# zynthbox/libzl

Measured on AMD Instinct MI355X. Metric: voice-samples/sec at 1024 voices x 256-frame blocks; % HBM roofline, higher is better.
Workload: dtype f32

## Files before the change

libzl_amd/build.py:

```python
from __future__ import annotations

import os
import shutil
import subprocess
import sys

ROOT = os.path.dirname(os.path.dirname(os.path.abspath(__file__)))
CSRC = os.path.join(ROOT, "libzl_amd", "csrc")
LIBDIR = os.path.join(ROOT, "libzl_amd", "lib")
LIB = os.path.join(LIBDIR, "libzlhip.so")

HIP_SOURCES = ["zl_kernels.hip", "zl_stretch.hip", "zl_overview.hip", "zl_decode.hip", "zl_engine.cpp", "zl_libzl.cpp", "zl_group.cpp"]
HEADERS = ["zl_types.h", "zl_arena.h", "zl_plan.h", "zl_order.h", "zl_pair.h", "zl_launch.h", "zl_render.h", "zl_kernels.h", "zl_host.h", "zl_sched.h", "zl_handoff.h", "zl_stretch.h", "zl_overview.h", "zl_decode.h", "zl_group.h", "zl_member.h",
           os.path.join("..", "..", "include", "zlhip.h"), os.path.join("..", "..", "include", "libzl_hotpath.h")]


def _hipcc() -> str:
    for cand in (os.environ.get("HIPCC"), shutil.which("hipcc"), "/opt/rocm/bin/hipcc"):
        if cand and os.path.exists(cand):
            return cand
    raise RuntimeError("hipcc not found (needed to build libzlhip.so for gfx950)")


def _stale(target: str, deps: list[str]) -> bool:
    if not os.path.exists(target):
        return True
    t = os.path.getmtime(target)
    return any(os.path.exists(d) and os.path.getmtime(d) > t for d in deps)


def build_variant(name: str, flags: list, verbose: bool = False) -> str:
    global LIB
    saved, LIB = LIB, os.path.join(LIBDIR, f"libzlhip_{name}.so")
    try:
        return _build_engine(False, verbose, list(flags))
    finally:
        LIB = saved


def build_engine(force: bool = False, verbose: bool = False, stamps: bool = False) -> str:
    global LIB
    if stamps:
        out = os.path.join(LIBDIR, "libzlhip_stamps.so")
        saved, LIB = LIB, out
        try:
            return _build_engine(force, verbose, ["-DZL_STAMPS"])
        finally:
            LIB = saved
    return _build_engine(force, verbose, [])


_INC = os.path.join("..", "..", "include")
SOURCE_DEPS = {
    "zl_kernels.hip": ["zl_types.h", "zl_plan.h", "zl_render.h", "zl_order.h", "zl_pair.h", "zl_launch.h", "zl_kernels.h"],
    "zl_stretch.hip": ["zl_types.h", "zl_stretch.h"],
    "zl_overview.hip": ["zl_types.h", "zl_overview.h"],
    "zl_decode.hip": ["zl_types.h", "zl_decode.h"],
    "zl_engine.cpp": ["zl_types.h", "zl_arena.h", "zl_plan.h", "zl_render.h", "zl_order.h", "zl_pair.h", "zl_launch.h", "zl_host.h", "zl_kernels.h", "zl_member.h", "zl_stretch.h", "zl_overview.h", "zl_decode.h", os.path.join(_INC, "zlhip.h")],
    "zl_group.cpp": ["zl_types.h", "zl_plan.h", "zl_order.h", "zl_pair.h", "zl_launch.h", "zl_host.h", "zl_kernels.h", "zl_member.h", "zl_group.h", os.path.join(_INC, "zlhip.h")],
    "zl_libzl.cpp": ["zl_render.h", "zl_types.h", "zl_sched.h", "zl_handoff.h", "zl_stretch.h", os.path.join(_INC, "zlhip.h"), os.path.join(_INC, "libzl_hotpath.h")],
}


def _write_kernel_resources(remarks: str, path: str) -> None:
    import re
    rows, cur = [], None
    for line in remarks.splitlines():
        m = re.search(r"remark:\s+Function Name: (\S+)", line)
        if m:
            cur = {"name": m.group(1)}
            rows.append(cur)
            continue
        m = re.search(r"remark:\s+(VGPRs|ScratchSize \[bytes/lane\]|Occupancy \[waves/SIMD\]|LDS Size \[bytes/block\]|VGPRs Spill): (\d+)", line)
        if m and cur is not None:
            cur[m.group(1).split(" ")[0] + ("Spill" if "Spill" in m.group(1) else "")] = int(m.group(2))
    with open(path, "w") as f:
        for r in rows:
            f.write(f"{r['name']} vgprs={r.get('VGPRs', -1)} scratch={r.get('ScratchSize', -1)} waves={r.get('Occupancy', -1)} lds={r.get('LDS', -1)} vgpr_spill={r.get('VGPRsSpill', -1)}\n")


def _build_engine(force: bool, verbose: bool, extra: list) -> str:
    names = [s for s in HIP_SOURCES if os.path.exists(os.path.join(CSRC, s))]
# ... 142 lines not shown


def build_pair_harness(force: bool = False) -> str:
    return _build_harness("zl_pair_host", "pair_host.cpp", ["zl_pair.h"], ["-Wall"], force)


def build_group_harness(force: bool = False) -> str:
    return _build_harness("zl_group_host", "group_host.cpp", ["zl_types.h", "zl_plan.h", "zl_host.h", "zl_group.h", _ZLHIP_H], _NO_CONTRACT + ["-Wall", "-Wno-unused-function"], force)


def build_overview_harness(force: bool = False) -> str:
    return _build_harness("zl_overview_host", "overview_host.cpp", ["zl_types.h", "zl_overview.h"], ["-Wall"], force)


def build_decode_harness(force: bool = False) -> str:
    return _build_harness("zl_decode_host", "decode_host.cpp", ["zl_types.h", "zl_decode.h"], _NO_CONTRACT + ["-Wall"], force)


def build_arena_harness(force: bool = False) -> str:
    return _build_harness("zl_arena_host", "arena_host.cpp", ["zl_types.h", "zl_stretch.h", "zl_arena.h"], ["-Wall"], force)


def build_launch_harness(force: bool = False) -> str:
    return _build_harness("zl_launch_host", "launch_host.cpp", ["zl_types.h", "zl_order.h", "zl_pair.h", "zl_launch.h"], ["-Wall", "-Wno-unused-function"], force)


if __name__ == "__main__":
    force = "--force" in sys.argv
    print(build_engine(force=force, verbose=True))
    print(build_oracle(force=force))
```

libzl_amd/csrc/zl_engine.cpp:

```cpp
#include <hip/hip_runtime.h>
#include <sys/resource.h>

#include <algorithm>
#include <atomic>
#include <cmath>
#include <cstdio>
#include <cstdlib>
#include <chrono>
#include <cstring>
#include <mutex>
#include <string>
#include <utility>
#include <vector>

#include "../../include/zlhip.h"
#include "zl_arena.h"
#include "zl_host.h"
#include "zl_kernels.h"
#include "zl_member.h"
#include "zl_order.h"
#include "zl_pair.h"
#include "zl_plan.h"
#include "zl_overview.h"
#include "zl_decode.h"
// ... 1347 lines not shown
        ZL_HIP(e, hipMemsetAsync(e->dTrace, 0xff, need * sizeof(int32_t), s));
        A.trace = 1; traceBase = e->dTrace; e->traceK = nblocks; e->traceN = nframes;
#ifdef ZL_STAMPS
        A.trace = 0;
#endif
    }

    static const int windowMulEnv = [] { const char *v = std::getenv("ZL_WINDOW_MUL"); const int m = v ? std::atoi(v) : 0; return m < 0 ? 0 : (m > 64 ? 64 : m); }();
    bool cheap = nframes >= 256;
    for (const ZlHostVoice &hv : e->hc.voices) if (hv.isPlaying && !hv.cheapPlan) { cheap = false; break; }
    int windowMul = windowMulEnv;
    if (windowMul == 0) windowMul = cheap ? 4 : 1;
    const size_t mul = e->maxGroups > 1 ? 1 : (size_t)windowMul;
    std::vector<std::pair<int, int>> &wins = e->wins;
    zlhip_engine::CallSlot &prev = e->slots[(e->callIndex + 1u) & 1u];
    const bool behindPrev = prev.inflight && hipEventQuery(prev.done) == hipErrorNotReady;
    const char *fw = std::getenv("ZL_FIRST_WINDOW_FRAMES");
    const int fwFrames = fw ? std::atoi(fw) : 0;
    zl_plan_windows(nblocks, nframes, e->windowBlocks, e->windowFrames, e->windowCap, mul, e->ps[1].hdr != nullptr, behindPrev, fw ? &fwFrames : nullptr, wins);
    const int nwin = (int)wins.size();
    const int phaseMode = [] { const char *v = std::getenv("ZL_K2_PHASE_ORDER"); return v ? std::atoi(v) : 1; }();
    const double loopFrames = phaseMode == 1 ? e->hc.phase_order_loop_frames() : INFINITY;
    const int pairMode = [] { const char *v = std::getenv("ZL_K2_PAIR"); return v ? std::atoi(v) : 1; }();
    const int stageNorun = [] { const char *v = std::getenv("ZL_K2_STAGE_NORUN"); return v ? (std::atoi(v) != 0 ? 1 : 0) : 1; }();
    const bool direct = e->bnc.sink.on && e->bnc.sink.hostDev && A.groups == 1;
    const ZlK2Switches &k2sw = zl_k2_switches();
    auto k2Launch = [&](int K, bool orderTable) {
        ZlK2In in;
        in.mode = A.mode; in.N = nframes; in.K = K; in.B = A.B; in.groups = A.groups; in.NB = A.NB;
        in.staged = A.staged; in.trace = A.trace; in.ongrid = A.ongrid; in.fan = fan_out_dev != nullptr; in.host_out = direct;
        in.order_mode = phaseMode; in.call_blocks = nblocks; in.bounce = e->bnc.sink.on; in.order_table = orderTable; in.loop_frames = loopFrames;
        in.pair_mode = pairMode; in.cheap = cheap;
        return zl_k2_launch(in, k2sw);
    };
    {
        size_t need = 0;
        for (const auto &wk : wins) { const ZlK2Launch L = k2Launch(wk.second, true); if (L.order) need = std::max(need, zl_order_ints((int)L.gz, wk.second, e->V)); }
        if (need > e->ps[0].orderInts || (e->ps[1].hdr != nullptr && need > e->ps[1].orderInts)) {
            ZlQuiesce quiet(e);
            for (auto &q : e->ps) {
                if (need <= q.orderInts || q.hdr == nullptr) continue;
                if (q.order) ZL_HIP(e, hipFree(q.order));
                q.order = nullptr; q.orderInts = 0;
                ZL_HIP(e, dalloc(&q.order, need));
                q.orderInts = need;
            }
        }
    }
    const bool overlap = e->ps[1].hdr != nullptr && (nwin > 1 || behindPrev || e->bnc.active);
    hipStream_t ps = overlap ? e->planStream : s;
    if (e->lastPlanStream && e->lastPlanStream != ps && e->lastPlanEvent) ZL_HIP(e, hipStreamWaitEvent(ps, e->lastPlanEvent, 0));
    if (nblocks == 1) { A.inline_clock = 1; A.clock0 = c.hClocks[0]; A.fuse_assemble = 1; }
    if (fan_out_dev) {
        for (int b = 0; b < A.B; ++b) c.hPass[b] = pass_params(fan_params[b]);
        ZL_HIP(e, hipMemcpyAsync(c.dPass, c.hPass, (size_t)A.B * sizeof(ZlPassParams), hipMemcpyHostToDevice, ps));
// ... 28 lines not shown
        if (w > 0) { Aw.n_op_ranges = 0; Aw.ops = nullptr; Aw.op_ranges = nullptr; Aw.n_clip_edits = 0; Aw.clip_edits = nullptr; }
        if (ps != s && q.used) ZL_HIP(e, hipStreamWaitEvent(ps, q.renderedEv, 0));
        ZL_KERNEL(e, zl_launch_apply_ops(Aw, ps));
        ZL_KERNEL(e, zl_launch_plan(Aw, e->forceSlow, ps));
        if (ps != s && e->asmStream && !Aw.fuse_assemble) {
            ZL_HIP(e, hipEventRecord(q.k1done, ps));
            ZL_HIP(e, hipStreamWaitEvent(e->asmStream, q.k1done, 0));
            ZL_KERNEL(e, zl_launch_assemble(Aw, e->asmStream));
            if (L.order) ZL_KERNEL(e, zl_launch_order(Aw, q.order, (int)L.gz, stageNorun, e->asmStream));
            ZL_HIP(e, hipEventRecord(q.planned, e->asmStream));
            ZL_HIP(e, hipStreamWaitEvent(s, q.planned, 0));
        } else {
            if (!Aw.fuse_assemble) ZL_KERNEL(e, zl_launch_assemble(Aw, ps));
            if (L.order) ZL_KERNEL(e, zl_launch_order(Aw, q.order, (int)L.gz, stageNorun, ps));
            if (ps != s) {
                ZL_HIP(e, hipEventRecord(q.planned, ps));
                ZL_HIP(e, hipStreamWaitEvent(s, q.planned, 0));
            }
        }
        const bool k3 = !L.scans_levels;
        if (direct) { Aw.host_out = e->bnc.sink.hostDev; Aw.host_fmt = e->bnc.sink.pcm ? 1 : 0; Aw.host_total = (long long)e->bnc.sink.totalFrames; Aw.host_k0 = 0; }
        const bool closes = fusedReports && w == nwin - 1;
        if (fusedReports) { Aw.fused_reports = 1; Aw.rep_gain = e->dGain; Aw.rep_host = c.hReportsDev; Aw.rep_host_gain = c.hGainDev; Aw.rep_host_stats = c.hStatsDev; }
        Aw.pair = (L.kernel == ZL_K2_PAIR_RENDER || L.kernel == ZL_K2_PAIR_PHASE_RENDER) ? 1 : 0;
        hipEvent_t k2stop = closes ? c.done : (e->profiling ? c.evK2[2 * (size_t)w + 1] : nullptr);
        ZL_KERNEL(e, zl_launch_render(Aw, L, s, e->profiling ? c.evK2[2 * (size_t)w] : nullptr, k2stop));
        if (k3) ZL_KERNEL(e, zl_launch_finalize(Aw, nullptr, s));
        if (e->bnc.sink.on && !direct) { int d_ = bounce_deliver_window(e, A.bus, 0, Aw.B, Aw.k0, Aw.K, nblocks, nframes, s); if (d_ != ZLHIP_OK) return d_; }
        if (e->ps[1].hdr != nullptr) {
            if (k2stop && !k3) q.renderedEv = k2stop;
            else { ZL_HIP(e, hipEventRecord(q.rendered, s)); q.renderedEv = q.rendered; }
            q.used = true;
        }
    }
    c.windows = nwin;
    if (ps != s) { ZL_HIP(e, hipEventRecord(e->evPlanTail, ps)); e->lastPlanEvent = e->evPlanTail; }
    else e->lastPlanEvent = c.done;
    e->lastPlanStream = ps;
    if (e->ps[1].hdr != nullptr) e->setPhase = (phase + (unsigned)nwin) & 1u;
    if (fusedReports) {
        if (e->profiling) c.profiled = true;
    } else {
        ZL_KERNEL(e, zl_launch_reports(c.dReports, e->V, e->dGain, c.hReportsDev, c.hGainDev, c.dStats, c.hStatsDev, s, e->profiling ? nullptr : c.done));
        if (e->profiling) { ZL_HIP(e, hipEventRecord(c.evEnd, s)); c.profiled = true; ZL_HIP(e, hipEventRecord(c.done, s)); }
    }
    c.inflight = true;
    if (s != e->stream) e->joins[0] = c.done;
// ... 666 lines not shown
```

libzl_amd/csrc/zl_kernels.hip:

```cpp
#include <hip/hip_runtime.h>
#include <hip/hip_ext.h>
#include <algorithm>
#include <cstddef>
#include "zl_types.h"
#include "zl_plan.h"
#include "zl_render.h"
#include "zl_order.h"
#include "zl_pair.h"
#include "zl_kernels.h"

static __device__ __forceinline__ void zl_apply_clip_edit(const ZlBatch &A, const ZlClipEdit *ed, int lane)
{
    static_assert(offsetof(ZlClip, slice_pos) == ZL_CLIP_HEAD_BYTES && sizeof(ZlClip) % 16 == 0 && offsetof(ZlClipEdit, c) % 16 == 0, "clip record layout");
    const int clip = ed->clip;
    const int n16 = ed->full ? (int)(sizeof(ZlClip) / 16) : ZL_CLIP_HEAD_BYTES / 16;
    const uint4 *src = reinterpret_cast<const uint4 *>(&ed->c);
    uint4 *dst = reinterpret_cast<uint4 *>(const_cast<ZlClip *>(A.clips) + clip);
    for (int w = lane; w < n16; w += 64) dst[w] = src[w];
}

__global__ void zl_k0_apply_ops(const ZlBatch A)
{
    const int opGroups = (A.n_op_ranges + 63) / 64;
    if ((int)blockIdx.x >= opGroups) {
        zl_apply_clip_edit(A, A.clip_edits + ((int)blockIdx.x - opGroups), (int)threadIdx.x);
        return;
    }
    const int i = blockIdx.x * blockDim.x + threadIdx.x;
    if (i >= A.n_op_ranges) return;
    const ZlOpRange rg = A.op_ranges[i];
    ZlVoiceState st = A.voices[rg.voice];
// ... 107 lines not shown
    ZlOrderKey key;
    if (s_key == INT_MAX || !zl_order_setup(A.runs[s_key], K, A.N, key)) {
        for (int k = tid; k < K; k += 256) out[k] = k;
        return;
    }
    for (int b = tid; b < key.nbkt; b += 256) s_hist[b] = 0;
    __syncthreads();
    for (int k = tid; k < K; k += 256) atomicAdd(&s_hist[zl_order_bucket(key, k)], 1);
    __syncthreads();
    const int per = (key.nbkt + 255) / 256, b0 = tid * per, b1 = b0 + per < key.nbkt ? b0 + per : key.nbkt;
    int sum = 0;
    for (int b = b0; b < b1; ++b) sum += s_hist[b];
    s_part[tid] = sum;
    __syncthreads();
    for (int off = 1; off < 256; off <<= 1) {
        const int t = tid >= off ? s_part[tid - off] : 0;
        __syncthreads();
        s_part[tid] += t;
        __syncthreads();
    }
    int run = s_part[tid] - sum;
    for (int b = b0; b < b1; ++b) { const int c = s_hist[b]; s_hist[b] = run; run += c; }
    __syncthreads();
    for (int k = tid; k < K; k += 256) out[atomicAdd(&s_hist[zl_order_bucket(key, k)], 1)] = k;
}

static __device__ __forceinline__ int zl_sample_to_peak_int(float x)
{
    const float v = 131072.0f * x;
    int r;
    asm("v_cvt_i32_f32_e64 %0, |%1|" : "=v"(r) : "v"(v));
    return r;
}

template <int CTRL, int ROWMASK>
static __device__ __forceinline__ int zl_dpp_i(int ident, int v) { return __builtin_amdgcn_update_dpp(ident, v, CTRL, ROWMASK, 0xf, false); }
static __device__ __forceinline__ int zl_wave_max_nonneg(int v)
{
    int t;
    t = zl_dpp_i<0xB1, 0xf>(0, v);  v = t > v ? t : v;
    t = zl_dpp_i<0x4E, 0xf>(0, v);  v = t > v ? t : v;
    t = zl_dpp_i<0x114, 0xf>(0, v); v = t > v ? t : v;
    t = zl_dpp_i<0x118, 0xf>(0, v); v = t > v ? t : v;
    t = zl_dpp_i<0x142, 0xa>(0, v); v = t > v ? t : v;
    t = zl_dpp_i<0x143, 0xc>(0, v); v = t > v ? t : v;
    return __builtin_amdgcn_readlane(v, 63);
}
// ... 1372 lines not shown

    if (A.fused_reports && A.k0 + k == A.Ktot - 1) {
        __syncthreads();
        for (int v = v0 + (int)threadIdx.x; v < v1; v += (int)blockDim.x) {
            const uint4 *src = reinterpret_cast<const uint4 *>(&A.reports[v]);
            uint4 a = src[0];
            const uint4 b = src[1];
            a.z = __hip_atomic_load(&A.reports[v].peak_bits, __ATOMIC_RELAXED, __HIP_MEMORY_SCOPE_AGENT);
            const float gn = __uint_as_float(a.z) * 0.5f;
            A.rep_gain[v] = gn;
            if (A.rep_host) { uint4 *dst = reinterpret_cast<uint4 *>(&A.rep_host[v]); dst[0] = a; dst[1] = b; A.rep_host_gain[v] = gn; }
        }
        if (bus == 0 && threadIdx.x == 0 && A.rep_host_stats) {
            const unsigned long long sb = A.stats->source_bytes, sl = A.stats->slow_blocks, af = A.stats->active_frames;
            A.rep_host_stats->source_bytes = sb; A.rep_host_stats->slow_blocks = sl; A.rep_host_stats->active_frames = af;
            A.stats->source_bytes = 0; A.stats->slow_blocks = 0; A.stats->active_frames = 0;
        }
    }
}

__global__ void __launch_bounds__(128, ZL_K2_PAIR_WAVES) zl_k2_pair_render(const ZlBatch A) { zl_k2_pair_body<false>(A); }
__global__ void __launch_bounds__(128, ZL_K2_PAIR_WAVES) zl_k2_pair_phase_render(const ZlBatch A) { zl_k2_pair_body<true>(A); }

static __device__ __forceinline__ void zl_k3_body(const ZlBatch &A, const float *bus_in, int k, int bus);
template <uint32_t MODE, bool WIDE>
__global__ void __launch_bounds__(256) __attribute__((amdgpu_waves_per_eu(2, 2))) zl_k_rt_loop(const ZlBatch A0, ZlRtShared *sh, ZlRtDev *dev, unsigned long long first_seq, unsigned long long idle_ticks,
                                                    float *gain_out, ZlReport *host_reports, float *host_gain, ZlOpRange *dev_ranges, int vw)
{
    __shared__ unsigned long long s_cmd[ZL_RT_CMD_WORDS + 1];
    __shared__ int s_go, s_last;
    __shared__ ZlClock s_clk0;
    __shared__ ZlPassParams s_pass;
    __shared__ uint32_t s_pass_seq;
    const int tid = threadIdx.x, lane = tid & 63;
    if (tid == 0) s_pass_seq = 0u;
    const int z = blockIdx.x, W = gridDim.x;
    const int vbeg = WIDE ? z * vw : z * A0.VPB, vend = WIDE ? vbeg + vw : vbeg + A0.VPB;
    unsigned long long last = first_seq;
    if (z == 0 && tid == 0) __hip_atomic_store(&sh->state, 1u, __ATOMIC_RELAXED, __HIP_MEMORY_SCOPE_SYSTEM);
    for (;;) {
        if (tid == 0) {
            int go = 0;
            if (z == 0) {
                const unsigned long long t0 = __builtin_amdgcn_s_memrealtime();
                for (;;) {
                    const unsigned long long q = __hip_atomic_load(&sh->cmd_seq, __ATOMIC_RELAXED, __HIP_MEMORY_SCOPE_SYSTEM);
// ... 470 lines not shown
int zl_launch_assemble(const ZlBatch &A, hipStream_t s)
{
    const int bpl = zl_k1c_blocks_per_lane(A);
    hipLaunchKernelGGL(zl_k1c_assemble, dim3((A.V + 63) / 64, (A.K + bpl - 1) / bpl), dim3(64), 0, s, A, bpl);
    ZL_LAUNCH_CHECK();
    return 0;
}

int zl_launch_order(const ZlBatch &A, int32_t *order, int nslots, int norun, hipStream_t s)
{
    hipLaunchKernelGGL(zl_k1o_order, dim3(nslots), dim3(256), 0, s, A, order, norun);
    ZL_LAUNCH_CHECK();
    return 0;
}

const ZlK2Switches &zl_k2_switches()
{
    static const ZlK2Switches sw = [] {
        ZlK2Switches w = zl_k2_env_switches();
        w.pair_lds = ZL_K2_PAIR_LDS;
        hipFuncAttributes fa;
        w.pair_static_lds = hipFuncGetAttributes(&fa, reinterpret_cast<const void *>(zl_k2_pair_render)) == hipSuccess ? (int)fa.sharedSizeBytes : ZL_K2_PAIR_LDS;
        w.st_ring = 4 * ZL_ST_D * ZL_ST_SLOT;
        return w;
    }();
    return sw;
}

static constexpr int zl_k2_key(int kernel, int bpw, bool st, int mode) { return ((kernel * 8 + bpw) * 2 + (st ? 1 : 0)) * 8 + mode; }

int zl_launch_render(const ZlBatch &A, const ZlK2Launch &L, hipStream_t s, hipEvent_t ev_start, hipEvent_t ev_stop)
{
    const dim3 grid(L.gx, L.gy, L.gz), block(L.threads);
    ZlBatch At = A;
    At.tail_from = L.tail_from; At.tail_split = L.tail_split; At.tail_nb = L.tail_nb;
    At.order = L.order ? A.order : nullptr;
#define ZL_GO(...) hipExtLaunchKernelGGL((__VA_ARGS__), grid, block, L.dyn_lds, s, ev_start, ev_stop, 0, At); break;
    switch (zl_k2_key(L.kernel, L.bpw, L.staged, (int)(A.mode & 7u))) {
#define ZL_CASE(M) \
    case zl_k2_key(ZL_K2_RENDER, 4, true, M):        ZL_GO(zl_k2_render<M, 4, true>) \
    case zl_k2_key(ZL_K2_RENDER, 2, true, M):        ZL_GO(zl_k2_render<M, 2, true>) \
    case zl_k2_key(ZL_K2_RENDER, 1, true, M):        ZL_GO(zl_k2_render<M, 1, true>) \
    case zl_k2_key(ZL_K2_RENDER, 4, false, M):       ZL_GO(zl_k2_render<M, 4, false>) \
    case zl_k2_key(ZL_K2_RENDER, 2, false, M):       ZL_GO(zl_k2_render<M, 2, false>) \
    case zl_k2_key(ZL_K2_PHASE_RENDER, 1, false, M): ZL_GO(zl_k2_phase_render<M>) \
    case zl_k2_key(ZL_K2_RENDER, 1, false, M):       ZL_GO(zl_k2_render<M, 1, false>)
        ZL_CASE(0) ZL_CASE(1) ZL_CASE(2) ZL_CASE(3) ZL_CASE(4) ZL_CASE(5) ZL_CASE(6) ZL_CASE(7)
#undef ZL_CASE
    case zl_k2_key(ZL_K2_PAIR_RENDER, 1, false, 0):       ZL_GO(zl_k2_pair_render)
    case zl_k2_key(ZL_K2_PAIR_PHASE_RENDER, 1, false, 0): ZL_GO(zl_k2_pair_phase_render)
    default: return (int)hipErrorInvalidValue;
    }
#undef ZL_GO
    ZL_LAUNCH_CHECK();
    return 0;
}

int zl_launch_rt_loop(const ZlBatch &A, void *mailbox_dev, void *dev_state, unsigned long long first_seq, unsigned long long idle_ticks, float *gain_out,
                      ZlReport *host_reports, float *host_gain, ZlOpRange *dev_ranges, int vw, int threads, hipStream_t s)
{
    ZlRtShared *sh = reinterpret_cast<ZlRtShared *>(mailbox_dev);
    ZlRtDev *dv = reinterpret_cast<ZlRtDev *>(dev_state);
    const bool wide = A.groups > 1;
    switch (A.mode & 7u) {
#define ZL_CASE(M) case M: \
        if (wide) hipLaunchKernelGGL((zl_k_rt_loop<M, true>), dim3(A.V / vw), dim3(threads), 0, s, A, sh, dv, first_seq, idle_ticks, gain_out, host_reports, host_gain, dev_ranges, vw); \
        else      hipLaunchKernelGGL((zl_k_rt_loop<M, false>), dim3(A.B), dim3(threads), 0, s, A, sh, dv, first_seq, idle_ticks, gain_out, host_reports, host_gain, dev_ranges, 0); \
        break;
        ZL_CASE(0) ZL_CASE(1) ZL_CASE(2) ZL_CASE(3) ZL_CASE(4) ZL_CASE(5) ZL_CASE(6) ZL_CASE(7)
#undef ZL_CASE
    }
    ZL_LAUNCH_CHECK();
    return 0;
// ... 113 lines not shown
```

libzl_amd/csrc/zl_launch.h:

```cpp
#pragma once
#include <stddef.h>
#include <stdint.h>
#include <stdlib.h>
#include <algorithm>
#include <utility>
#include <vector>
#include "zl_order.h"
#include "zl_pair.h"

inline int zl_whole_waves(int nframes) { return nframes < 256 ? ((nframes + 63) & ~63) : 256; }

inline int zl_k2_narrow_buses(int nblocks, int groups, int VPB, int B, int nframes)
{
    if (nblocks > 1 && groups == 1 && VPB <= 64 && (VPB % 8) == 0 && nframes <= 256) return std::max(1, std::min(128 / VPB, B));
    return 1;
}

#define ZL_K2_MAX_WINDOW 60000
inline void zl_plan_windows(int nblocks, int nframes, int windowBlocks, size_t windowFrames, int windowCap, size_t mul, bool twoSets,
                            bool behindPrev, const int *firstWindowFrames, std::vector<std::pair<int, int>> &wins)
{
    int W = windowBlocks > 0 ? windowBlocks : (int)std::max<size_t>(1, std::min<size_t>(mul * windowFrames / (size_t)nframes, (size_t)1 << 30));
    W = std::min(W, windowCap);
    W = std::min(W, (1 << 30) / nframes);
    W = std::min(W, ZL_K2_MAX_WINDOW);
    wins.clear();
    if (nblocks <= W || !twoSets || behindPrev) {
        for (int k0 = 0; k0 < nblocks; k0 += W) wins.push_back({k0, std::min(W, nblocks - k0)});
        return;
    }
    int size = std::min(W, std::max(1, (firstWindowFrames ? *firstWindowFrames : (int)std::min<size_t>(windowFrames / 4, (size_t)1 << 28)) / nframes));
    for (int k0 = 0; k0 < nblocks;) {
        const int n = std::min(size, nblocks - k0);
        wins.push_back({k0, n});
        k0 += n;
        size = W;
    }
}

struct ZlK2Switches {
    int tail = 1;
    int tail_min = 2048;
    int pad = -1;
    int pad_hermite = -1;
    int pair_pad = -1;
    int pair_static_lds = 0;
    int pair_lds = 0;
    int st_ring = 0;
};

inline ZlK2Switches zl_k2_env_switches()
{
    auto env = [](const char *name, int dflt) { const char *e = getenv(name); return e ? atoi(e) : dflt; };
    ZlK2Switches w;
    w.tail = env("ZL_K2_TAIL", w.tail);
    if (getenv("ZL_K2_TAIL_MIN_BLOCKS")) w.tail_min = std::max(8, env("ZL_K2_TAIL_MIN_BLOCKS", 0));
    w.pad = env("ZL_K2_LDS_PAD", w.pad);
    w.pad_hermite = env("ZL_K2_LDS_PAD_HERMITE", w.pad_hermite);
    w.pair_pad = env("ZL_K2_PAIR_LDS_PAD", w.pair_pad);
    return w;
}

struct ZlK2In {
    uint32_t mode;
    int N, K, B, groups, NB;
    int staged, trace, ongrid;
    bool fan, host_out;
    int order_mode, call_blocks;
    bool bounce, order_table;
    double loop_frames;
    int pair_mode;
    bool cheap;
};

enum ZlK2Kernel { ZL_K2_RENDER, ZL_K2_PHASE_RENDER, ZL_K2_PAIR_RENDER, ZL_K2_PAIR_PHASE_RENDER };

struct ZlK2Launch {
    int kernel;
    int bpw; bool staged;
    unsigned gx, gy, gz, threads, dyn_lds;
    int tail_from, tail_split, tail_nb;
    bool order;
    bool scans_levels;
};

inline ZlK2Launch zl_k2_launch(const ZlK2In &in, const ZlK2Switches &sw)
{
    const int N = in.N, K = in.K, NB = in.NB;
    ZlK2Launch L{};
    L.bpw = ((N == 64 || N == 128) && K > 1) ? 256 / N : 1;
    L.threads = L.bpw > 1 ? 256u : (unsigned)zl_whole_waves(N);
    L.gx = L.bpw > 1 ? 1u : ((unsigned)N + L.threads - 1) / L.threads;
    L.gy = (unsigned)((K + L.bpw - 1) / L.bpw);
    L.gz = (unsigned)(NB > 1 ? (in.B + NB - 1) / NB : in.B * in.groups);
    L.scans_levels = in.groups == 1 && L.gx == 1;
    L.tail_from = 0; L.tail_split = 1; L.tail_nb = NB;
    const bool pair = zl_pair_window(in.pair_mode, zl_pair_shape(in.mode, N, K, NB, in.groups, in.staged, in.trace, in.fan, in.host_out, in.ongrid), in.cheap);
    L.order = in.order_table && zl_order_window(in.order_mode, zl_order_shape(in.groups, in.staged, in.call_blocks, N), in.bounce, N, K, in.loop_frames);
    if (pair) {
        L.kernel = L.order ? ZL_K2_PAIR_PHASE_RENDER : ZL_K2_PAIR_RENDER;
        L.threads = 128;
        L.dyn_lds = (unsigned)(sw.pair_pad >= 0 ? sw.pair_pad : std::max(0, sw.pair_lds - sw.pair_static_lds));
        return L;
    }
    L.kernel = L.order ? ZL_K2_PHASE_RENDER : ZL_K2_RENDER;
    L.staged = in.staged && K > 1 && L.threads == 256;
    if (sw.tail && L.bpw == 1 && NB > 1 && NB == in.B && L.gz == 1 && L.gx == 1 && !L.staged && K >= sw.tail_min) {
        const int split = (NB % 4 == 0) ? 4 : (NB % 2 == 0) ? 2 : 1;
        if (split > 1) {
            const int T = std::min(K / 4, 640);
            L.tail_from = K - T; L.tail_split = split; L.tail_nb = NB / split;
            L.gy = (unsigned)(L.tail_from + T * split);
        }
    }
    const int pad = (in.mode & ZL_MODE_HERMITE) ? (sw.pad_hermite >= 0 ? sw.pad_hermite : 0) : (sw.pad >= 0 ? sw.pad : 10240);
    L.dyn_lds = (unsigned)(L.staged ? sw.st_ring : L.bpw > 1 ? 0 : pad);
    return L;
}
```

Baseline: 2100 billion.

## Add two-lap pair render kernel sharing voice constants across adjacent ordered blocks

Adds a new render kernel in which each workgroup renders two adjacent blocks from the phase-order table, one per wave. It stages voice plans for both blocks and, when both chunks are on-grid with the same mono/stereo class, mixes them in one pass that reuses the same pan constants. The aim is to halve the number of workgroups and cut repeated staging and LDS traffic per block. The order-scatter loop now places keys in synchronized rounds of 256 so that adjacent slots keep a deterministic order, which adds barriers to that loop. The kernel is on by default when the pair and order paths are both chosen and the call spans at least two loop lengths. The fallback path parks accumulators in LDS and may cost extra.

```diff
diff --git a/libzl_amd/build.py b/libzl_amd/build.py
--- a/libzl_amd/build.py
+++ b/libzl_amd/build.py
@@ -11,7 +11,7 @@
 LIB = os.path.join(LIBDIR, "libzlhip.so")
 
 HIP_SOURCES = ["zl_kernels.hip", "zl_stretch.hip", "zl_overview.hip", "zl_decode.hip", "zl_engine.cpp", "zl_libzl.cpp", "zl_group.cpp"]
-HEADERS = ["zl_types.h", "zl_arena.h", "zl_plan.h", "zl_order.h", "zl_pair.h", "zl_launch.h", "zl_render.h", "zl_kernels.h", "zl_host.h", "zl_sched.h", "zl_handoff.h", "zl_stretch.h", "zl_overview.h", "zl_decode.h", "zl_group.h", "zl_member.h",
+HEADERS = ["zl_types.h", "zl_arena.h", "zl_plan.h", "zl_order.h", "zl_pair.h", "zl_lap.h", "zl_launch.h", "zl_render.h", "zl_kernels.h", "zl_host.h", "zl_sched.h", "zl_handoff.h", "zl_stretch.h", "zl_overview.h", "zl_decode.h", "zl_group.h", "zl_member.h",
            os.path.join("..", "..", "include", "zlhip.h"), os.path.join("..", "..", "include", "libzl_hotpath.h")]
 
 
@@ -52,12 +52,12 @@
 
 _INC = os.path.join("..", "..", "include")
 SOURCE_DEPS = {
-    "zl_kernels.hip": ["zl_types.h", "zl_plan.h", "zl_render.h", "zl_order.h", "zl_pair.h", "zl_launch.h", "zl_kernels.h"],
+    "zl_kernels.hip": ["zl_types.h", "zl_plan.h", "zl_render.h", "zl_order.h", "zl_pair.h", "zl_lap.h", "zl_launch.h", "zl_kernels.h"],
     "zl_stretch.hip": ["zl_types.h", "zl_stretch.h"],
     "zl_overview.hip": ["zl_types.h", "zl_overview.h"],
     "zl_decode.hip": ["zl_types.h", "zl_decode.h"],
-    "zl_engine.cpp": ["zl_types.h", "zl_arena.h", "zl_plan.h", "zl_render.h", "zl_order.h", "zl_pair.h", "zl_launch.h", "zl_host.h", "zl_kernels.h", "zl_member.h", "zl_stretch.h", "zl_overview.h", "zl_decode.h", os.path.join(_INC, "zlhip.h")],
-    "zl_group.cpp": ["zl_types.h", "zl_plan.h", "zl_order.h", "zl_pair.h", "zl_launch.h", "zl_host.h", "zl_kernels.h", "zl_member.h", "zl_group.h", os.path.join(_INC, "zlhip.h")],
+    "zl_engine.cpp": ["zl_types.h", "zl_arena.h", "zl_plan.h", "zl_render.h", "zl_order.h", "zl_pair.h", "zl_lap.h", "zl_launch.h", "zl_host.h", "zl_kernels.h", "zl_member.h", "zl_stretch.h", "zl_overview.h", "zl_decode.h", os.path.join(_INC, "zlhip.h")],
+    "zl_group.cpp": ["zl_types.h", "zl_plan.h", "zl_order.h", "zl_pair.h", "zl_lap.h", "zl_launch.h", "zl_host.h", "zl_kernels.h", "zl_member.h", "zl_group.h", os.path.join(_INC, "zlhip.h")],
     "zl_libzl.cpp": ["zl_render.h", "zl_types.h", "zl_sched.h", "zl_handoff.h", "zl_stretch.h", os.path.join(_INC, "zlhip.h"), os.path.join(_INC, "libzl_hotpath.h")],
 }
 
@@ -246,7 +246,11 @@
 
 
 def build_launch_harness(force: bool = False) -> str:
-    return _build_harness("zl_launch_host", "launch_host.cpp", ["zl_types.h", "zl_order.h", "zl_pair.h", "zl_launch.h"], ["-Wall", "-Wno-unused-function"], force)
+    return _build_harness("zl_launch_host", "launch_host.cpp", ["zl_types.h", "zl_order.h", "zl_pair.h", "zl_lap.h", "zl_launch.h"], ["-Wall", "-Wno-unused-function"], force)
+
+
+def build_lap_harness(force: bool = False) -> str:
+    return _build_harness("zl_lap_host", "lap_host.cpp", ["zl_types.h", "zl_order.h", "zl_pair.h", "zl_lap.h", "zl_launch.h"], ["-Wall", "-Wno-unused-function"], force)
 
 
 if __name__ == "__main__":
diff --git a/libzl_amd/csrc/zl_engine.cpp b/libzl_amd/csrc/zl_engine.cpp
--- a/libzl_amd/csrc/zl_engine.cpp
+++ b/libzl_amd/csrc/zl_engine.cpp
@@ -1393,6 +1393,7 @@
     const int phaseMode = [] { const char *v = std::getenv("ZL_K2_PHASE_ORDER"); return v ? std::atoi(v) : 1; }();
     const double loopFrames = phaseMode == 1 ? e->hc.phase_order_loop_frames() : INFINITY;
     const int pairMode = [] { const char *v = std::getenv("ZL_K2_PAIR"); return v ? std::atoi(v) : 1; }();
+    const int lapMode = [] { const char *v = std::getenv("ZL_K2_LAP"); return v ? std::atoi(v) : ZL_K2_LAP_DEFAULT; }();
     const int stageNorun = [] { const char *v = std::getenv("ZL_K2_STAGE_NORUN"); return v ? (std::atoi(v) != 0 ? 1 : 0) : 1; }();
     const bool direct = e->bnc.sink.on && e->bnc.sink.hostDev && A.groups == 1;
     const ZlK2Switches &k2sw = zl_k2_switches();
@@ -1401,7 +1402,7 @@
         in.mode = A.mode; in.N = nframes; in.K = K; in.B = A.B; in.groups = A.groups; in.NB = A.NB;
         in.staged = A.staged; in.trace = A.trace; in.ongrid = A.ongrid; in.fan = fan_out_dev != nullptr; in.host_out = direct;
         in.order_mode = phaseMode; in.call_blocks = nblocks; in.bounce = e->bnc.sink.on; in.order_table = orderTable; in.loop_frames = loopFrames;
-        in.pair_mode = pairMode; in.cheap = cheap;
+        in.pair_mode = pairMode; in.cheap = cheap; in.lap_mode = lapMode;
         return zl_k2_launch(in, k2sw);
     };
     {
@@ -1476,7 +1477,7 @@
         if (direct) { Aw.host_out = e->bnc.sink.hostDev; Aw.host_fmt = e->bnc.sink.pcm ? 1 : 0; Aw.host_total = (long long)e->bnc.sink.totalFrames; Aw.host_k0 = 0; }
         const bool closes = fusedReports && w == nwin - 1;
         if (fusedReports) { Aw.fused_reports = 1; Aw.rep_gain = e->dGain; Aw.rep_host = c.hReportsDev; Aw.rep_host_gain = c.hGainDev; Aw.rep_host_stats = c.hStatsDev; }
-        Aw.pair = (L.kernel == ZL_K2_PAIR_RENDER || L.kernel == ZL_K2_PAIR_PHASE_RENDER) ? 1 : 0;
+        Aw.pair = (L.kernel == ZL_K2_PAIR_RENDER || L.kernel == ZL_K2_PAIR_PHASE_RENDER || L.kernel == ZL_K2_LAP_RENDER) ? 1 : 0;
         hipEvent_t k2stop = closes ? c.done : (e->profiling ? c.evK2[2 * (size_t)w + 1] : nullptr);
         ZL_KERNEL(e, zl_launch_render(Aw, L, s, e->profiling ? c.evK2[2 * (size_t)w] : nullptr, k2stop));
         if (k3) ZL_KERNEL(e, zl_launch_finalize(Aw, nullptr, s));
diff --git a/libzl_amd/csrc/zl_kernels.hip b/libzl_amd/csrc/zl_kernels.hip
--- a/libzl_amd/csrc/zl_kernels.hip
+++ b/libzl_amd/csrc/zl_kernels.hip
@@ -7,6 +7,7 @@
 #include "zl_render.h"
 #include "zl_order.h"
 #include "zl_pair.h"
+#include "zl_lap.h"
 #include "zl_kernels.h"
 
 static __device__ __forceinline__ void zl_apply_clip_edit(const ZlBatch &A, const ZlClipEdit *ed, int lane)
@@ -160,7 +161,12 @@
     int run = s_part[tid] - sum;
     for (int b = b0; b < b1; ++b) { const int c = s_hist[b]; s_hist[b] = run; run += c; }
     __syncthreads();
-    for (int k = tid; k < K; k += 256) out[atomicAdd(&s_hist[zl_order_bucket(key, k)], 1)] = k;
+    static_assert(ZL_LAP_ROUND == 256, "a round is the workgroup's lanes");
+    for (int k0 = 0; k0 < K; k0 += ZL_LAP_ROUND) {
+        const int k = k0 + tid;
+        if (k < K) out[atomicAdd(&s_hist[zl_order_bucket(key, k)], 1)] = k;
+        __syncthreads();
+    }
 }
 
 static __device__ __forceinline__ int zl_sample_to_peak_int(float x)
@@ -1579,6 +1585,226 @@
 __global__ void __launch_bounds__(128, ZL_K2_PAIR_WAVES) zl_k2_pair_render(const ZlBatch A) { zl_k2_pair_body<false>(A); }
 __global__ void __launch_bounds__(128, ZL_K2_PAIR_WAVES) zl_k2_pair_phase_render(const ZlBatch A) { zl_k2_pair_body<true>(A); }
 
+#ifndef ZL_K2_U_LAP
+#define ZL_K2_U_LAP 8
+#endif
+#define ZL_K2_LAP_CHUNK 64
+#define ZL_K2_LAP_WAVES 4
+#define ZL_K2_LAP_LDS 18432
+template <bool MONO, int U>
+static __device__ __forceinline__ void zl_k2_chunk_ongrid_lap(const ZlVoiceConst *s_vc, const ZlUnit *s_ua, const ZlUnit *s_ub, int c0, int f0,
+                                                               float &aL0, float &aR0, float &aL1, float &aR1, float &bL0, float &bR0, float &bL1, float &bR1)
+{
+    zl_f4a8 da[MONO ? 1 : U], db[MONO ? 1 : U];
+    zl_f2   ea[MONO ? U : 1], eb[MONO ? U : 1];
+    const uint32_t ob = zl_k2_ongrid_offset((uint32_t)f0 << (MONO ? 2 : 3));
+    zl_f2 pan[U];
+#pragma unroll
+    for (int u = 0; u < U; ++u) {
+        const uint64_t srca = zl_k2_ongrid_base(s_ua, c0 + u), srcb = zl_k2_ongrid_base(s_ub, c0 + u);
+        if (MONO) { ea[u] = zl_k2_ongrid_load<zl_f2a4b>(srca, ob); eb[u] = zl_k2_ongrid_load<zl_f2a4b>(srcb, ob); }
+        else      { da[u] = zl_k2_ongrid_load<zl_f4a8>(srca, ob);  db[u] = zl_k2_ongrid_load<zl_f4a8>(srcb, ob); }
+    }
+    __builtin_amdgcn_sched_barrier(0);
+#pragma unroll
+    for (int u = 0; u < U; ++u) pan[u] = *reinterpret_cast<const zl_f2 *>(&s_vc[c0 + u].lpan);
+    zl_f2 a0 = {aL0, aR0}, a1 = {aL1, aR1}, b0 = {bL0, bR0}, b1 = {bL1, bR1};
+#pragma unroll
+    for (int u = 0; u < U; ++u) {
+        if (MONO) {
+            zl_mix_acc_ongrid_pk<1>(a0, ea[u], pan[u]);
+            zl_mix_acc_ongrid_pk<2>(a1, ea[u], pan[u]);
+            zl_mix_acc_ongrid_pk<1>(b0, eb[u], pan[u]);
+            zl_mix_acc_ongrid_pk<2>(b1, eb[u], pan[u]);
+        } else {
+            zl_mix_acc_ongrid_pk<0>(a0, __builtin_shufflevector(da[u], da[u], 0, 1), pan[u]);
+            zl_mix_acc_ongrid_pk<0>(a1, __builtin_shufflevector(da[u], da[u], 2, 3), pan[u]);
+            zl_mix_acc_ongrid_pk<0>(b0, __builtin_shufflevector(db[u], db[u], 0, 1), pan[u]);
+            zl_mix_acc_ongrid_pk<0>(b1, __builtin_shufflevector(db[u], db[u], 2, 3), pan[u]);
+        }
+    }
+    aL0 = a0.x; aR0 = a0.y; aL1 = a1.x; aR1 = a1.y;
+    bL0 = b0.x; bR0 = b0.y; bL1 = b1.x; bR1 = b1.y;
+}
+
+static __device__ __forceinline__ void zl_k2_lap_chunk_seq(const ZlBatch &A, const ZlBlockPlan *s_plan, const ZlVoiceConst *s_vc, const int *s_cls, const ZlUnit *s_unit,
+                                                           int cc, int c0, int vb, int f0, int k, bool wantPeak, float &accL0, float &accR0, float &accL1, float &accR1)
+{
+    constexpr uint32_t MODE = 0;
+    constexpr int U = ZL_K2_U, UP = ZL_K2_U_PAIR;
+    if (cc == 0) return;
+    if ((cc & 132) == 132) {
+#pragma unroll
+        for (int h = 0; h < U; h += UP) {
+            if (wantPeak) {
+                if (cc & 16) zl_k2_chunk_ongrid_pair<true, UP, true>(A, s_vc, s_unit, c0 + h, vb, f0, accL0, accR0, accL1, accR1);
+                else         zl_k2_chunk_ongrid_pair<false, UP, true>(A, s_vc, s_unit, c0 + h, vb, f0, accL0, accR0, accL1, accR1);
+            }
+            else if (cc & 16) zl_k2_chunk_ongrid_pair<true, UP, false>(A, s_vc, s_unit, c0 + h, vb, f0, accL0, accR0, accL1, accR1);
+            else              zl_k2_chunk_ongrid_pair<false, UP, false>(A, s_vc, s_unit, c0 + h, vb, f0, accL0, accR0, accL1, accR1);
+        }
+        return;
+    }
+#pragma nounroll
+    for (int h = 0; h < 2; ++h) {
+        const int fc = f0 + h;
+        const double fd = (double)fc;
+        float accL = h ? accL1 : accL0, accR = h ? accR1 : accR0;
+        if ((cc & 124) == 100)      zl_k2_chunk_simple<MODE, false, true, true, U>(A, s_plan, s_vc, s_unit, c0, vb, fc, fd, wantPeak, accL, accR);
+        else if ((cc & 92) == 68)   zl_k2_chunk_simple<MODE, false, false, true, U>(A, s_plan, s_vc, s_unit, c0, vb, fc, fd, wantPeak, accL, accR);
+        else if ((cc & 28) == 4)    zl_k2_chunk_simple<MODE, false, false, false, U>(A, s_plan, s_vc, s_unit, c0, vb, fc, fd, wantPeak, accL, accR);
+        else if ((cc & 20) == 4)    zl_k2_chunk_simple<MODE, true, false, false, U>(A, s_plan, s_vc, s_unit, c0, vb, fc, fd, wantPeak, accL, accR);
+        else if ((cc & 124) == 116) zl_k2_chunk_simple_mono<MODE, false, true, true, U>(A, s_plan, s_vc, s_unit, c0, vb, fc, fd, wantPeak, accL, accR);
+        else if ((cc & 92) == 84)   zl_k2_chunk_simple_mono<MODE, false, false, true, U>(A, s_plan, s_vc, s_unit, c0, vb, fc, fd, wantPeak, accL, accR);
+        else if ((cc & 28) == 20)   zl_k2_chunk_simple_mono<MODE, false, false, false, U>(A, s_plan, s_vc, s_unit, c0, vb, fc, fd, wantPeak, accL, accR);
+        else if ((cc & 20) == 20)   zl_k2_chunk_simple_mono<MODE, true, false, false, U>(A, s_plan, s_vc, s_unit, c0, vb, fc, fd, wantPeak, accL, accR);
+        else {
+            constexpr int H = U / 2;
+            const size_t pbase = (size_t)k * A.V + vb;
+            for (int q = 0; q < U; q += H) {
+                if (cc & 2) zl_k2_chunk<MODE, true, H>(A, s_plan, s_vc, s_cls, c0 + q, pbase, vb, fc, wantPeak, accL, accR);
+                else        zl_k2_chunk<MODE, false, H>(A, s_plan, s_vc, s_cls, c0 + q, pbase, vb, fc, wantPeak, accL, accR);
+            }
+        }
+        if (h) { accL1 = accL; accR1 = accR; } else { accL0 = accL; accR0 = accR; }
+    }
+}
+
+static __device__ __forceinline__ void zl_k2_lap_finish(const ZlBatch &A, int k, int bus, int f0, float accL0, float accR0, float accL1, float accR1, int (*s_pk)[4], float (*s_sq)[4])
+{
+    const int N = A.N;
+    const long long KN = (long long)A.Ktot * N;
+    float *outL = A.bus + (long long)bus * (A.bus_stride ? A.bus_stride : 2 * KN) + (long long)(A.k0 + k) * N;
+    float *outR = outL + (A.ch_stride ? A.ch_stride : KN);
+    const bool written1 = f0 + 2 < N;
+    outL[f0 + 1] = accL0; outR[f0 + 1] = accR0;
+    if (written1) { outL[f0 + 2] = accL1; outR[f0 + 2] = accR1; }
+    if (f0 == 0)  { outL[0] = 0.0f; outR[0] = 0.0f; }
+    if (A.levels) {
+        const float bL = written1 ? accL1 : 0.0f, bR = written1 ? accR1 : 0.0f;
+        const int pa = zl_sample_to_peak_int(accL0), pb = zl_sample_to_peak_int(bL), pc = zl_sample_to_peak_int(accR0), pd = zl_sample_to_peak_int(bR);
+        int pkL[2], pkR[2]; float sqL[2], sqR[2];
+        zl_wave_levels4_pair(pb > pa ? pb : pa, pd > pc ? pd : pc, accL0 * accL0 + bL * bL, accR0 * accR0 + bR * bR, pkL, pkR, sqL, sqR);
+        const int w = (int)(threadIdx.x >> 6) * 2;
+        if ((threadIdx.x & 63) == 0) {
+            s_pk[0][w] = pkL[0]; s_pk[1][w] = pkR[0]; s_sq[0][w] = sqL[0]; s_sq[1][w] = sqR[0];
+            s_pk[0][w + 1] = pkL[1]; s_pk[1][w + 1] = pkR[1]; s_sq[0][w + 1] = sqL[1]; s_sq[1][w + 1] = sqR[1];
+        }
+        __syncthreads();
+        if (threadIdx.x == 0) {
+            ZlBlockLevels lv; lv.peak_l = 0; lv.peak_r = 0; lv.sumsq_l = 0.0f; lv.sumsq_r = 0.0f;
+            for (int t = 0; t < 4; ++t) {
+                lv.peak_l = s_pk[0][t] > lv.peak_l ? s_pk[0][t] : lv.peak_l;
+                lv.peak_r = s_pk[1][t] > lv.peak_r ? s_pk[1][t] : lv.peak_r;
+                lv.sumsq_l += s_sq[0][t]; lv.sumsq_r += s_sq[1][t];
+            }
+            A.levels[(size_t)k * A.B + bus] = lv;
+        }
+    }
+}
+
+__global__ void __launch_bounds__(128, ZL_K2_LAP_WAVES) zl_k2_lap_render(const ZlBatch A)
+{
+    constexpr uint32_t MODE = 0;
+    constexpr int U = ZL_K2_U, UL = ZL_K2_U_LAP, CH = ZL_K2_LAP_CHUNK;
+    static_assert(UL == U || 2 * UL == U, "the two-lap chunk walks a chunk class of U voices whole or in halves");
+    static_assert(CH == 64, "a pass is one wave's voices per lap");
+    __shared__ ZlBlockPlan  s_plan[2][CH];
+    __shared__ ZlVoiceConst s_vc[CH];
+    __shared__ int s_cls[2][CH];
+    __shared__ int s_chunk[2][CH / U];
+    __shared__ ZlUnit s_unit[2][CH];
+    __shared__ int   s_pk[2][2][4];
+    __shared__ float s_sq[2][2][4];
+    __shared__ float s_park[4][128];
+
+    const int f0 = 2 * (int)threadIdx.x;
+    const unsigned by = blockIdx.y, bz = blockIdx.z;
+    const int ky = (int)gridDim.y, xq = ky >> 3, xr = ky & 7, xx = (int)(by & 7u);
+    const int ys = xx * xq + (xx < xr ? xx : xr) + (int)(by >> 3);
+    int e0, e1;
+    const bool two = zl_lap_slots(A.K, ys, e0, e1) == 2;
+    const int ka = A.order[(size_t)bz * A.K + e0], kb = A.order[(size_t)bz * A.K + e1];
+    __builtin_assume(ka >= 0 && ka < 65536 && kb >= 0 && kb < 65536);
+    const int bus = (int)bz;
+    const int v0 = bus * A.VPB, vlim = (bus + 1) * A.VPB;
+    const int v1 = (v0 + A.G < vlim) ? v0 + A.G : vlim;
+    const bool wantPeakA = __builtin_amdgcn_readfirstlane((int)(A.k0 + ka == A.Ktot - 1)) != 0;
+    const bool wantPeakB = __builtin_amdgcn_readfirstlane((int)(two && A.k0 + kb == A.Ktot - 1)) != 0;
+    const bool fast = two && !wantPeakA && !wantPeakB;
+    const int32_t *dead_tail = A.order + zl_order_tail_dead((int)gridDim.z, A.K, 0);
+    const int run_end = A.order[zl_order_tail_run_end((int)gridDim.z, A.K, (int)bz)];
+    const int wlap = (int)(threadIdx.x >> 6);
+    const int kw = __builtin_amdgcn_readfirstlane(wlap ? kb : ka);
+    const bool norunw = __builtin_amdgcn_readfirstlane((int)(kw >= run_end)) != 0;
+
+    float aL0 = 0.0f, aR0 = 0.0f, aL1 = 0.0f, aR1 = 0.0f, bL0 = 0.0f, bR0 = 0.0f, bL1 = 0.0f, bR1 = 0.0f;
+    for (int vb = v0; vb < v1; vb += CH) {
+        const int nv = (v1 - vb < CH) ? v1 - vb : CH;
+        if (vb != v0) __syncthreads();
+        {
+            const int i = (int)(threadIdx.x & 63u);
+            ZlVoiceConst vc;
+            ZlBlockPlan pl;
+            if (norunw) zl_k2_stage_load<false>(A, kw, vb, i, nv, vc, pl, dead_tail);
+            else        zl_k2_stage_load<true>(A, kw, vb, i, nv, vc, pl, nullptr);
+            const int cls = zl_k2_stage_class<MODE>(A, vc, pl);
+            s_unit[wlap][i] = zl_unit_record<MODE>(A, vc, pl, cls);
+            if (wlap == 0) s_vc[i] = vc;
+            s_plan[wlap][i] = pl;
+            s_cls[wlap][i] = cls;
+            zl_k2_stage_chunks<U>(cls, i, s_chunk[wlap]);
+        }
+        __syncthreads();
+        for (int c0 = 0; c0 < nv; c0 += U) {
+            const int cca = __builtin_amdgcn_readfirstlane(s_chunk[0][c0 / U]), ccb = __builtin_amdgcn_readfirstlane(s_chunk[1][c0 / U]);
+            if (fast && (cca & 132) == 132 && (ccb & 132) == 132 && ((cca ^ ccb) & 16) == 0) {
+#pragma unroll
+                for (int h = 0; h < U; h += UL) {
+                    if (cca & 16) zl_k2_chunk_ongrid_lap<true, UL>(s_vc, s_unit[0], s_unit[1], c0 + h, f0, aL0, aR0, aL1, aR1, bL0, bR0, bL1, bR1);
+                    else          zl_k2_chunk_ongrid_lap<false, UL>(s_vc, s_unit[0], s_unit[1], c0 + h, f0, aL0, aR0, aL1, aR1, bL0, bR0, bL1, bR1);
+                }
+            } else {
+                const int t = (int)threadIdx.x;
+                float cL0 = aL0, cR0 = aR0, cL1 = aL1, cR1 = aR1;
+                s_park[0][t] = bL0; s_park[1][t] = bR0; s_park[2][t] = bL1; s_park[3][t] = bR1;
+#pragma nounroll
+                for (int lap = 0; lap < 2; ++lap) {
+                    if (lap == 0 || two)
+                        zl_k2_lap_chunk_seq(A, s_plan[lap], s_vc, s_cls[lap], s_unit[lap], lap ? ccb : cca, c0, vb, f0, lap ? kb : ka, lap ? wantPeakB : wantPeakA,
+                                            cL0, cR0, cL1, cR1);
+                    const float p0 = s_park[0][t], p1 = s_park[1][t], p2 = s_park[2][t], p3 = s_park[3][t];
+                    s_park[0][t] = cL0; s_park[1][t] = cR0; s_park[2][t] = cL1; s_park[3][t] = cR1;
+                    cL0 = p0; cR0 = p1; cL1 = p2; cR1 = p3;
+                }
+                aL0 = cL0; aR0 = cR0; aL1 = cL1; aR1 = cR1;
+                bL0 = s_park[0][t]; bR0 = s_park[1][t]; bL1 = s_park[2][t]; bR1 = s_park[3][t];
+            }
+        }
+    }
+
+    zl_k2_lap_finish(A, ka, bus, f0, aL0, aR0, aL1, aR1, s_pk[0], s_sq[0]);
+    if (two) zl_k2_lap_finish(A, kb, bus, f0, bL0, bR0, bL1, bR1, s_pk[1], s_sq[1]);
+
+    if (A.fused_reports && (A.k0 + ka == A.Ktot - 1 || A.k0 + kb == A.Ktot - 1)) {
+        __syncthreads();
+        for (int v = v0 + (int)threadIdx.x; v < v1; v += (int)blockDim.x) {
+            const uint4 *src = reinterpret_cast<const uint4 *>(&A.reports[v]);
+            uint4 ra = src[0];
+            const uint4 rb = src[1];
+            ra.z = __hip_atomic_load(&A.reports[v].peak_bits, __ATOMIC_RELAXED, __HIP_MEMORY_SCOPE_AGENT);
+            const float gn = __uint_as_float(ra.z) * 0.5f;
+            A.rep_gain[v] = gn;
+            if (A.rep_host) { uint4 *dst = reinterpret_cast<uint4 *>(&A.rep_host[v]); dst[0] = ra; dst[1] = rb; A.rep_host_gain[v] = gn; }
+        }
+        if (bus == 0 && threadIdx.x == 0 && A.rep_host_stats) {
+            const unsigned long long sb = A.stats->source_bytes, sl = A.stats->slow_blocks, af = A.stats->active_frames;
+            A.rep_host_stats->source_bytes = sb; A.rep_host_stats->slow_blocks = sl; A.rep_host_stats->active_frames = af;
+            A.stats->source_bytes = 0; A.stats->slow_blocks = 0; A.stats->active_frames = 0;
+        }
+    }
+}
+
 static __device__ __forceinline__ void zl_k3_body(const ZlBatch &A, const float *bus_in, int k, int bus);
 template <uint32_t MODE, bool WIDE>
 __global__ void __launch_bounds__(256) __attribute__((amdgpu_waves_per_eu(2, 2))) zl_k_rt_loop(const ZlBatch A0, ZlRtShared *sh, ZlRtDev *dev, unsigned long long first_seq, unsigned long long idle_ticks,
@@ -2095,6 +2321,8 @@
         hipFuncAttributes fa;
         w.pair_static_lds = hipFuncGetAttributes(&fa, reinterpret_cast<const void *>(zl_k2_pair_render)) == hipSuccess ? (int)fa.sharedSizeBytes : ZL_K2_PAIR_LDS;
         w.st_ring = 4 * ZL_ST_D * ZL_ST_SLOT;
+        w.lap_lds = ZL_K2_LAP_LDS;
+        w.lap_static_lds = hipFuncGetAttributes(&fa, reinterpret_cast<const void *>(zl_k2_lap_render)) == hipSuccess ? (int)fa.sharedSizeBytes : ZL_K2_LAP_LDS;
         return w;
     }();
     return sw;
@@ -2122,6 +2350,7 @@
 #undef ZL_CASE
     case zl_k2_key(ZL_K2_PAIR_RENDER, 1, false, 0):       ZL_GO(zl_k2_pair_render)
     case zl_k2_key(ZL_K2_PAIR_PHASE_RENDER, 1, false, 0): ZL_GO(zl_k2_pair_phase_render)
+    case zl_k2_key(ZL_K2_LAP_RENDER, 1, false, 0):        ZL_GO(zl_k2_lap_render)
     default: return (int)hipErrorInvalidValue;
     }
 #undef ZL_GO
diff --git a/libzl_amd/csrc/zl_lap.h b/libzl_amd/csrc/zl_lap.h
--- /dev/null
+++ b/libzl_amd/csrc/zl_lap.h
@@ -0,0 +1,37 @@
+#pragma once
+#include "zl_order.h"
+
+ZL_HD inline int zl_lap_pairs(int K) { return (K + 1) / 2; }
+
+ZL_HD inline int zl_lap_slots(int K, int y, int &e0, int &e1)
+{
+    e0 = 2 * y;
+    e1 = 2 * y + 1 < K ? 2 * y + 1 : e0;
+    return 2 * y + 1 < K ? 2 : 1;
+}
+
+ZL_HD inline bool zl_lap_window(int sw, bool pair, bool order, int nframes, int K, double loopFrames)
+{
+    if (!(pair && order && K >= 2)) return false;
+    return sw == 2 || (sw == 1 && (double)K * nframes >= 2.0 * loopFrames);
+}
+
+#ifndef ZL_K2_LAP_DEFAULT
+#define ZL_K2_LAP_DEFAULT 1
+#endif
+
+#define ZL_LAP_ROUND 256
+
+inline void zl_lap_place_host(const ZlOrderKey *key, int K, const int *tie, int *hist, int *order)
+{
+    if (!key) { for (int k = 0; k < K; ++k) order[k] = k; return; }
+    for (int b = 0; b < key->nbkt; ++b) hist[b] = 0;
+    for (int k = 0; k < K; ++k) ++hist[zl_order_bucket(*key, k)];
+    int run = 0;
+    for (int b = 0; b < key->nbkt; ++b) { const int c = hist[b]; hist[b] = run; run += c; }
+    for (int k0 = 0; k0 < K; k0 += ZL_LAP_ROUND)
+        for (int j = 0; j < ZL_LAP_ROUND; ++j) {
+            const int k = k0 + (tie ? tie[j] : j);
+            if (k < K) order[hist[zl_order_bucket(*key, k)]++] = k;
+        }
+}
diff --git a/libzl_amd/csrc/zl_launch.h b/libzl_amd/csrc/zl_launch.h
--- a/libzl_amd/csrc/zl_launch.h
+++ b/libzl_amd/csrc/zl_launch.h
@@ -7,6 +7,7 @@
 #include <vector>
 #include "zl_order.h"
 #include "zl_pair.h"
+#include "zl_lap.h"
 
 inline int zl_whole_waves(int nframes) { return nframes < 256 ? ((nframes + 63) & ~63) : 256; }
 
@@ -47,6 +48,9 @@
     int pair_static_lds = 0;
     int pair_lds = 0;
     int st_ring = 0;
+    int lap_pad = -1;
+    int lap_static_lds = 0;
+    int lap_lds = 0;
 };
 
 inline ZlK2Switches zl_k2_env_switches()
@@ -58,6 +62,7 @@
     w.pad = env("ZL_K2_LDS_PAD", w.pad);
     w.pad_hermite = env("ZL_K2_LDS_PAD_HERMITE", w.pad_hermite);
     w.pair_pad = env("ZL_K2_PAIR_LDS_PAD", w.pair_pad);
+    w.lap_pad = env("ZL_K2_LAP_LDS_PAD", w.lap_pad);
     return w;
 }
 
@@ -71,9 +76,10 @@
     double loop_frames;
     int pair_mode;
     bool cheap;
+    int lap_mode = 0;
 };
 
-enum ZlK2Kernel { ZL_K2_RENDER, ZL_K2_PHASE_RENDER, ZL_K2_PAIR_RENDER, ZL_K2_PAIR_PHASE_RENDER };
+enum ZlK2Kernel { ZL_K2_RENDER, ZL_K2_PHASE_RENDER, ZL_K2_PAIR_RENDER, ZL_K2_PAIR_PHASE_RENDER, ZL_K2_LAP_RENDER };
 
 struct ZlK2Launch {
     int kernel;
@@ -98,8 +104,14 @@
     const bool pair = zl_pair_window(in.pair_mode, zl_pair_shape(in.mode, N, K, NB, in.groups, in.staged, in.trace, in.fan, in.host_out, in.ongrid), in.cheap);
     L.order = in.order_table && zl_order_window(in.order_mode, zl_order_shape(in.groups, in.staged, in.call_blocks, N), in.bounce, N, K, in.loop_frames);
     if (pair) {
+        L.threads = 128;
+        if (zl_lap_window(in.lap_mode, pair, L.order, N, K, in.loop_frames)) {
+            L.kernel = ZL_K2_LAP_RENDER;
+            L.gy = (unsigned)zl_lap_pairs(K);
+            L.dyn_lds = (unsigned)(sw.lap_pad >= 0 ? sw.lap_pad : std::max(0, sw.lap_lds - sw.lap_static_lds));
+            return L;
+        }
         L.kernel = L.order ? ZL_K2_PAIR_PHASE_RENDER : ZL_K2_PAIR_RENDER;
-        L.threads = 128;
         L.dyn_lds = (unsigned)(sw.pair_pad >= 0 ? sw.pair_pad : std::max(0, sw.pair_lds - sw.pair_static_lds));
         return L;
     }
```

Result: faster. 2219 billion (median of 6 runs) (+5.7%).
